# PranjalSahu/tensorflow_distributed

Hardware: AMD Instinct MI355X
Metric: images/sec (whole node) MNIST CNN DP at 1/2/4/8 MI355X; step-time scaling (higher is better)
Workload: dtype bf16; 1 GPU; global_batch=128, per_gpu_batch=128, parallelism=dp1, grad_allreduce=bf16, hipgraph=True, steps_per_graph=20, dp_transport=none, force_dp=False, zero1_fc1=False, fc_grads=bf16

## Files before the change

### csrc/kernels/mnist.hip

```cpp
#include "../common.h"

#include "../gemm.h"
#include "../gemm256.h"
#include "../mnist_layout.h"
#include "../tfd_kernels.h"
#include "../mnist_tail.h"

#include <algorithm>
#include <stdexcept>

constexpr int GEMM_RS = 2;
constexpr int FDX_BK_ = 128;
constexpr int FDW_BK_ = 64;
constexpr int FC1_BK_ = 32;

namespace tfd {
using namespace mnist;

namespace {

__device__ __forceinline__ int data_row(const int* perm, const int64_t* step, int n_data, int B, int b) {
  if (!perm) return b;
  const int64_t s = *step;
  return perm[(int)((s * (int64_t)B + b) % (int64_t)n_data)];
// ... 437 lines not shown
  for (int c = 0; c < NCLS; ++c) part[(q * 64 + r) * NCLS + c] = acc[c];
  __syncthreads();
  for (int i = t; i < OUTG_ROWS * NCLS; i += 256) {
    const int rr = i / NCLS, mm = blk * OUTG_ROWS + rr;
    if (mm <= HID) {
      const size_t o = OFF_OUT + (size_t)mm * NCLS + (i - rr * NCLS);
      const float g =
          part[i] + part[OUTG_ROWS * NCLS + i] + part[2 * OUTG_ROWS * NCLS + i] + part[3 * OUTG_ROWS * NCLS + i];
      if (a.gbf_a) {
        a.gbf_a[o] = f2bf_bits(g);
      } else {
        a.grad[o] = g;
      }
    }
  }
}

struct OnesRowBuf {
  static constexpr bool KC = false;
  const uint16_t* __restrict__ x;
  int k_lim;
  uint32_t nbytes;
  __device__ __forceinline__ uint4 operator()(int mn, int k) const {
    const uint4 v = buf_ld(x, nbytes, (uint32_t)k * FEAT + mn, k < k_lim && mn < FEAT);
    return (mn == FEAT && k < k_lim) ? make_uint4(0x3F80u, 0u, 0u, 0u) : v;
  }
};
static_assert(FEAT % 8 == 0, "the ones row starts a fresh 8-element chunk");

constexpr int FDW_BM = 64, FDW_BN = 64, FDW_BK = FDW_BK_;
constexpr int FDW_PITCH = FDW_BN + 4;
__device__ __forceinline__ void fc1_dw_store(f32x4 (&acc)[2][2], float* cs, float* out, uint16_t* outbf, int m0,
                                             int n0, int M) {
  const int tid = threadIdx.x, lane = tid & 63, w = tid >> 6, wm = w >> 1, wn = w & 1;
#pragma unroll
  for (int i = 0; i < 2; ++i)
#pragma unroll
    for (int j = 0; j < 2; ++j)
#pragma unroll
      for (int r = 0; r < 4; ++r)
        cs[(wm * 32 + 16 * i + 4 * (lane >> 4) + r) * FDW_PITCH + wn * 32 + 16 * j + (lane & 15)] = acc[i][j][r];
  __syncthreads();
#pragma unroll
  for (int q = tid; q < FDW_BM * FDW_BN / 8; q += 256) {
    const int row = q >> 3, ch = q & 7, m = m0 + row;
    if (m >= M) continue;
    const f32x4 lo = *reinterpret_cast<const f32x4*>(cs + row * FDW_PITCH + ch * 8);
    const f32x4 hi = *reinterpret_cast<const f32x4*>(cs + row * FDW_PITCH + ch * 8 + 4);
    const size_t o = (size_t)m * HID + n0 + ch * 8;
    if (outbf) {
      *reinterpret_cast<uint4*>(outbf + o) =
          make_uint4(pack_bf2(lo[0], lo[1]), pack_bf2(lo[2], lo[3]), pack_bf2(hi[0], hi[1]), pack_bf2(hi[2], hi[3]));
    } else {
      *reinterpret_cast<f32x4*>(out + o) = lo;
      *reinterpret_cast<f32x4*>(out + o + 4) = hi;
    }
  }
}
template <class LA, class LB>
__device__ __forceinline__ void fc1_dw_tile(const MnistStepArgs& a, const LA& la, const LB& lb, int m0, int n0, int K,
                                            bf16* smem) {
  f32x4 acc[2][2];
  gemm_mainloop<FDW_BM, FDW_BN, FDW_BK, 2, 2, LA, LB, GEMM_RS>(la, lb, m0, n0, 0, K, smem, acc);
  fc1_dw_store(acc, reinterpret_cast<float*>(smem), a.grad + OFF_WD1, a.gbf_a ? a.gbf_a + OFF_WD1 : nullptr, m0, n0,
               FEAT + 1);
}
__device__ __forceinline__ void fc1_dw_block(const MnistStepArgs& a, int bx, int by, bf16* smem) {
  OnesRowBuf la{a.p2, a.B, (uint32_t)((int64_t)a.B * FEAT * 2)};
  DenseLoaderX<false> lb{a.dh, HID, HID, a.B};
  fc1_dw_tile(a, la, lb, by * FDW_BM, bx * FDW_BN, a.B, smem);
}

constexpr int FDX_BM = 32, FDX_BN = 64, FDX_BK = FDX_BK_, FDX_BN2 = 32;
template <int BN>
__device__ __forceinline__ void fc1_dx_unpool_store(const MnistStepArgs& a, f32x4 (&acc)[FDX_BM / 32][BN / 32],
                                                    float* cs, int m0, int n0) {
  constexpr int PITCH = BN + 4, CPR = BN / 8;
  const int tid = threadIdx.x, lane = tid & 63, w = tid >> 6, wm = w >> 1, wn = w & 1;
  constexpr int WTM = FDX_BM / 2, WTN = BN / 2;
  const int b = tid / CPR, cc = tid % CPR, m = m0 + b;
  const bool live = b < FDX_BM && m < a.B;
  const size_t xo = (size_t)(live ? m : 0) * FEAT + n0 + cc * 8;
  const uint4 pv = *reinterpret_cast<const uint4*>(a.p2 + xo);
  const uint2 iv = *reinterpret_cast<const uint2*>(a.idx2 + xo);
#pragma unroll
  for (int i = 0; i < WTM / 16; ++i)
#pragma unroll
    for (int j = 0; j < WTN / 16; ++j)
#pragma unroll
      for (int r = 0; r < 4; ++r)
        cs[(wm * WTM + 16 * i + 4 * (lane >> 4) + r) * PITCH + wn * WTN + 16 * j + (lane & 15)] = acc[i][j][r];
  __syncthreads();
  if (!live) return;
  const f32x4 lo = *reinterpret_cast<const f32x4*>(cs + b * PITCH + cc * 8);
  const f32x4 hi = *reinterpret_cast<const f32x4*>(cs + b * PITCH + cc * 8 + 4);
  const float v[8] = {lo[0], lo[1], lo[2], lo[3], hi[0], hi[1], hi[2], hi[3]};
  const uint32_t pw[4] = {pv.x, pv.y, pv.z, pv.w};
  uint32_t g[8];
#pragma unroll
  for (int j = 0; j < 8; ++j) {
    const uint32_t p = (pw[j >> 1] >> (16 * (j & 1))) & 0xFFFFu;
    g[j] = p != 0 ? (uint32_t)f2bf_bits(v[j]) : 0u;
  }
  const int pp = n0 >> 6, c0 = (n0 & 63) + cc * 8, ph = pp / 7, pwx = pp - ph * 7;
  const uint32_t iw[2] = {iv.x, iv.y};
#pragma unroll
  for (int wi = 0; wi < 4; ++wi) {
    uint32_t o[4];
#pragma unroll
    for (int q = 0; q < 4; ++q) {
      const uint32_t i0 = (iw[q >> 1] >> (16 * (q & 1))) & 0xFFu, i1 = (iw[q >> 1] >> (16 * (q & 1) + 8)) & 0xFFu;
      o[q] = (i0 == (uint32_t)wi ? g[2 * q] : 0u) | (i1 == (uint32_t)wi ? g[2 * q + 1] << 16 : 0u);
    }
    const int oh = 2 * ph + (wi >> 1), ow = 2 * pwx + (wi & 1);
    *reinterpret_cast<uint4*>(a.dz2 + ((size_t)(m * 14 + oh) * 14 + ow) * 64 + c0) = make_uint4(o[0], o[1], o[2], o[3]);
  }
}
constexpr int FDX_RS = 1, FDX_RS_ALONE = 2;
constexpr int FDXD_BK = 64, FDXD_S = 4;
constexpr int FDXD_A = FDX_BM * FDXD_BK * 2, FDXD_B = FDX_BN * FDXD_BK * 2, FDXD_STAGE = FDXD_A + FDXD_B;
constexpr int FDXD_SMEM = FDXD_S * FDXD_STAGE;
constexpr int FDXD_NK = HID / FDXD_BK;
static_assert(FDX_BM == 32 && FDX_BN == 64 && FDXD_NK >= FDXD_S, "fc1 dX DMA ring geometry");
__device__ __forceinline__ void fdxd_stage(const DenseKC& sa, const DenseKC& sb, char* img, int m0, int n0, int k0,
                                           int w, int l) {
#if defined(__HIP_DEVICE_COMPILE__)
  {
    const int row = w * 8 + (l >> 3);
    __builtin_amdgcn_raw_ptr_buffer_load_lds(sa.rsrc(), (__attribute__((address_space(3))) void*)(img + w * 1024), 16,
                                             sa.off(m0 + row, k0 + kc_slot(row, l & 7) * 8), 0, 0, 0);
  }
#pragma unroll
  for (int i = 0; i < 2; ++i) {
    const int ins = 2 * w + i, row = ins * 8 + (l >> 3);
    __builtin_amdgcn_raw_ptr_buffer_load_lds(sb.rsrc(), (__attribute__((address_space(3))) void*)(img + FDXD_A + ins * 1024),
                                             16, sb.off(n0 + row, k0 + kc_slot(row, l & 7) * 8), 0, 0, 0);
  }
#else
  (void)sa; (void)sb; (void)img; (void)m0; (void)n0; (void)k0; (void)w; (void)l;
#endif
}
__device__ __forceinline__ void fc1_dx_block_dma(const MnistStepArgs& a, int bx, int by, char* smem) {
  const DenseKC sa{a.dh, HID, a.B, HID};
  const DenseKC sb{a.pbf + OFF_WD1, HID, FEAT, HID};
  const int tid = threadIdx.x, l = tid & 63, w = tid >> 6, wm = w >> 1, wn = w & 1;
  const int m0 = by * FDX_BM, n0 = bx * FDX_BN;
  f32x4 acc[1][2] = {{f32x4{0.f, 0.f, 0.f, 0.f}, f32x4{0.f, 0.f, 0.f, 0.f}}};
#pragma unroll
  for (int s = 0; s < FDXD_S - 1; ++s) fdxd_stage(sa, sb, smem + s * FDXD_STAGE, m0, n0, s * FDXD_BK, w, l);
  for (int t = 0; t < FDXD_NK; ++t) {
    const int after = min(FDXD_S - 2, FDXD_NK - 1 - t);
    if (after == 2) asm volatile("s_waitcnt vmcnt(6)" ::: "memory");
    else if (after == 1) asm volatile("s_waitcnt vmcnt(3)" ::: "memory");
    else asm volatile("s_waitcnt vmcnt(0)" ::: "memory");
    __syncthreads();
    if (t + FDXD_S - 1 < FDXD_NK)
      fdxd_stage(sa, sb, smem + ((t + FDXD_S - 1) % FDXD_S) * FDXD_STAGE, m0, n0, (t + FDXD_S - 1) * FDXD_BK, w, l);
    const char* As = smem + (t % FDXD_S) * FDXD_STAGE;
    const char* Bs = As + FDXD_A;
#pragma unroll
    for (int ks = 0; ks < 2; ++ks) {
      const int ch = 4 * ks + (l >> 4);
      const int ra = 16 * wm + (l & 15);
      const bf16x8 af = *reinterpret_cast<const bf16x8*>(As + ra * 128 + (kc_slot(ra, ch) << 4));
#pragma unroll
      for (int j = 0; j < 2; ++j) {
        const int rb = 32 * wn + 16 * j + (l & 15);
        const bf16x8 bf = *reinterpret_cast<const bf16x8*>(Bs + rb * 128 + (kc_slot(rb, ch) << 4));
        acc[0][j] = mfma16x16x32(af, bf, acc[0][j]);
      }
    }
  }
  __syncthreads();
  fc1_dx_unpool_store<FDX_BN>(a, acc, reinterpret_cast<float*>(smem), m0, n0);
}

template <int BN = FDX_BN, int RS = FDX_RS>
__device__ __forceinline__ void fc1_dx_block(const MnistStepArgs& a, int bx, int by, bf16* smem) {
  DenseLoaderX<true> la{a.dh, HID, a.B, HID};
  DenseLoaderX<true> lb{a.pbf + OFF_WD1, HID, FEAT, HID};
  f32x4 acc[FDX_BM / 32][BN / 32];
  gemm_mainloop<FDX_BM, BN, FDX_BK, 2, 2, decltype(la), decltype(lb), RS>(la, lb, by * FDX_BM, bx * BN, 0, HID, smem,
                                                                          acc);
  fc1_dx_unpool_store<BN>(a, acc, reinterpret_cast<float*>(smem), by * FDX_BM, bx * BN);
}

constexpr int FDW_GX = HID / FDW_BN, FDW_GY = (FEAT + 1 + FDW_BM - 1) / FDW_BM;
constexpr int FDX_GX = FEAT / FDX_BN;
constexpr int FDX_GX2 = FEAT / FDX_BN2;
static_assert(FEAT % FDX_BN == 0 && FEAT % FDX_BN2 == 0, "fc1 dX tiles cover the 3136 features exactly");
__device__ __forceinline__ void fdx_tile(int j, int gx, int gy, int& bx, int& by) {
  const int full = (gx * gy) / (8 * gy) * (8 * gy);
  const int T = j < full ? (j & 7) * (full >> 3) + (j >> 3) : j;
  bx = T / gy;
  by = T - bx * gy;
}
__global__ __launch_bounds__(256) void fc1_bwd(MnistStepArgs a, int n_dx, int part) {
  extern __shared__ __attribute__((aligned(16))) char smem_raw[];
  int id = blockIdx.x;
// ... 37 lines not shown
  const int m = blk * OUTS_ROWS + r;
  const int B = a.B, WB = a.sfb_world * B;
  const int per = (WB + OUTS_GROUPS - 1) / OUTS_GROUPS, k0 = min(WB, q * per), k1 = min(WB, k0 + per);
  const int64_t hoff = (int64_t)B * HID, doff = 2 * (int64_t)B * HID;
  float acc[NCLS];
#pragma unroll
  for (int c = 0; c < NCLS; ++c) acc[c] = 0.f;
  if (m <= HID) {
    for (int kb = k0; kb < k1; kb += OUTS_LB) {
      float hv[OUTS_LB];
      const float* dl[OUTS_LB];
#pragma unroll
      for (int u = 0; u < OUTS_LB; ++u) {
        const int k = min(kb + u, k1 - 1), rk = k / B, row = k - rk * B;
        const uint16_t* slot = a.sfb_dr + rk * a.sfb_rs;
        hv[u] = (kb + u < k1) ? (m < HID ? bf2f(slot[hoff + (int64_t)row * HID + m]) : 1.f) : 0.f;
        dl[u] = reinterpret_cast<const float*>(slot + doff) + row * NCLS;
      }
#pragma unroll
      for (int u = 0; u < OUTS_LB; ++u)
#pragma unroll
        for (int c = 0; c < NCLS; ++c) acc[c] = fmaf(hv[u], dl[u][c], acc[c]);
    }
  }
#pragma unroll
  for (int c = 0; c < NCLS; ++c) part[(q * OUTS_ROWS + r) * NCLS + c] = acc[c];
  __syncthreads();
  if (t < OUTS_ROWS * NCLS) {
    const int rr = t / NCLS, c = t - rr * NCLS, mm = blk * OUTS_ROWS + rr;
    float g = 0.f;
#pragma unroll
    for (int qq = 0; qq < OUTS_GROUPS; ++qq) g += part[(qq * OUTS_ROWS + rr) * NCLS + c];
    if (mm <= HID) {
      const size_t o = OFF_OUT + (size_t)mm * NCLS + c;
      if (a.gbf_a) a.gbf_a[o] = f2bf_bits(g);
      else a.grad[o] = g;
    }
  }
}

__device__ __forceinline__ int xcd_grouped_tile(int b, int first, int n) {
  const int x = b & 7;
  const int first_x = first + ((x - first) & 7);
  return x * (n >> 3) + ((b - first_x) >> 3);
}


constexpr int C2D_ROWS = 11, C2D_COLS = 20, C2D_PLANE = 224;
constexpr int C2B_NT = 256;
__device__ __forceinline__ const bf16* c2d_w(const bf16* wt, int rr, int ch) {
  return wt + rr * 64 + ((ch ^ (rr & 7)) << 3);
}
__device__ __forceinline__ uint4 buf_ld_so(const uint16_t* base, uint32_t nbytes, uint32_t voff, uint32_t soff) {
  const __amdgpu_buffer_rsrc_t r = __builtin_amdgcn_make_buffer_rsrc((void*)base, (short)0, (int)nbytes, 0x00020000);
  const i32x4v v = __builtin_amdgcn_raw_buffer_load_b128(r, (int)voff, (int)soff, 0);
  return make_uint4((uint32_t)v[0], (uint32_t)v[1], (uint32_t)v[2], (uint32_t)v[3]);
}
#ifndef C2D_TPS
#define C2D_TPS 5
#endif
constexpr int C2D_NST = 25 / C2D_TPS, C2D_WSTAGE = C2D_TPS * 32 * 64;
static_assert(C2D_NST * C2D_TPS == 25 && C2D_WSTAGE % 512 == 0, "whole W2 stages of 1-KB DMA rows");
constexpr int C2D_SMEM = (8 * C2D_PLANE * 8 + 2 * C2D_WSTAGE) * 2;
static_assert(2 * C2D_SMEM <= 160 * 1024, "two conv2_bwd_lds blocks share a CU (the launch's point)");
static_assert(C2D_PLANE * 16 % 256 == 0 && C2D_PLANE >= C2D_ROWS * C2D_COLS, "dz2 plane");
constexpr int C2D_X_OFF = 8 * C2D_PLANE * 8 * 2;
constexpr int C2D_Z_OFF = C2D_X_OFF;
constexpr int C2D_XS_OFF = C2D_Z_OFF + 448 * 32 * 2;
constexpr int C2D_T_END = C2D_XS_OFF + 5 * 18 * 40 * 2;
static_assert(C2D_T_END <= C2D_SMEM && C2D_XS_OFF % 16 == 0 && (C2D_T_END - C2D_Z_OFF) % 16 == 0, "MFMA tail LDS");
__device__ __forceinline__ int c1w_dz(int px, int c) {
  return px * 32 + (((c >> 3) ^ (2 * ((px >> 3) & 1))) << 3) + (c & 7);
}
#define C2D_STAMP(k)                                                                                     \
  do {                                                                                                   \
    if (TFD_STAMP && a.dbg && threadIdx.x == 0) a.dbg[5 * a.B * 8 + bid * 8 + (k)] = (int64_t)__builtin_amdgcn_s_memtime(); \
  } while (0)
__device__ __forceinline__ void conv2_dgrad_body(const MnistStepArgs& a, const int bid) {
  C2D_STAMP(0);
  extern __shared__ __attribute__((aligned(16))) char smem_raw[];
  bf16* img = (bf16*)smem_raw;
  bf16* wt = img + 8 * C2D_PLANE * 8;
  const int b = bid >> 1, h = bid & 1, t = threadIdx.x;
  const uint16_t* src = a.dz2 + (size_t)b * 196 * 64;
  const uint16_t* wsrc = a.pbf + OFF_WC2;
  const RowPre xr = data_row_pre(a, b);
  auto wdma = [&](int st) {
    constexpr int NI = C2D_WSTAGE / 512;
    static_assert(NI % (C2B_NT / 64) == 0, "whole DMA instructions per wave");
    const int wv = t >> 6, ln = t & 63;
    const uint16_t* s0 = wsrc + st * C2D_WSTAGE;
    bf16* d0 = wt + (st & 1) * C2D_WSTAGE;
#pragma unroll
    for (int k = 0; k < NI / (C2B_NT / 64); ++k) {
      const int ii = wv + (C2B_NT / 64) * k, p = ii * 64 + ln, rr = p >> 3, sl = p & 7;
      __builtin_amdgcn_global_load_lds((const void*)(s0 + rr * 64 + ((sl ^ (rr & 7)) << 3)),
                                       (__attribute__((address_space(3))) void*)(d0 + ii * 64 * 8), 16, 0, 0);
    }
  };
  {
    constexpr int CI = 8 * C2D_PLANE, NI = CI / C2B_NT;
    static_assert(CI % C2B_NT == 0, "whole image chunks per thread");
    wdma(0);
    wdma(1);
    uint4 vi[NI];
#pragma unroll
    for (int j = 0; j < NI; ++j) {
      const int i = t + C2B_NT * j, ch = i / C2D_PLANE, px = i - ch * C2D_PLANE;
      const int r = px / C2D_COLS + 7 * h - 2, c = px % C2D_COLS - 2;
      vi[j] = buf_ld(src, 196 * 64 * 2, (uint32_t)((r * 14 + c) * 64 + ch * 8),
                     px < C2D_ROWS * C2D_COLS && (unsigned)r < 14u && (unsigned)c < 14u);
    }
#pragma unroll
    for (int j = 0; j < NI; ++j) *reinterpret_cast<uint4*>(img + (t + C2B_NT * j) * 8) = vi[j];
  }
  C2D_STAMP(1);
  const int lane = t & 63, w = t >> 6, g = lane >> 4, mt0 = w;
  const int two = (mt0 + 4 < 7);
  float xpre[4];
  uint32_t p1pre[2][2][4];
  uint32_t ipb[2][2][4];
  {
    const float* xrow = a.data + (size_t)data_row_use(a, xr, b) * 784;
#pragma unroll
    for (int q = 0; q < 4; ++q) {
      const int i = 4 * t + q, r = i >> 5, c = i & 31;
      xpre[q] = (r >= 2 && r < 30 && c >= 2 && c < 30) ? xrow[(r - 2) * 28 + c - 2] : 0.f;
    }
  }
#pragma unroll
  for (int j = 0; j < 2; ++j)
#pragma unroll
    for (int nt = 0; nt < 2; ++nt)
#pragma unroll
      for (int r = 0; r < 4; ++r) {
        const int x = min(4 * g + r, 13), n = nt * 16 + (lane & 15), ih = 7 * h + min(mt0 + 4 * j, 6);
        p1pre[j][nt][r] = a.p1[((size_t)b * 196 + ih * 14 + x) * 32 + n];
        ipb[j][nt][r] = a.idx1[((size_t)b * 196 + ih * 14 + x) * 32 + n];
      }
  __syncthreads();
  C2D_STAMP(2);
  const int iw = lane & 15, nl = lane & 15;
  f32x4 acc[2][2];
#pragma unroll
  for (int j = 0; j < 2; ++j) acc[j][0] = acc[j][1] = f32x4{0.f, 0.f, 0.f, 0.f};
  {
    const bf16* a0 = img + ((mt0 + 4) * C2D_COLS + iw + 4) * 8 + g * C2D_PLANE * 8 - (4 * C2D_COLS + 4) * 8;
    const bf16* a1 = a0 + 4 * C2D_COLS * 8;
    const bf16* bw[2][2] = {{c2d_w(wt, nl, g), c2d_w(wt, 16 + nl, g)}, {c2d_w(wt, nl, g + 4), c2d_w(wt, 16 + nl, g + 4)}};
    bf16x8 fb[2][2], fa[2][2];
    auto ld = [&](int st, int slot) {
      const int tap = st >> 1, sk = st & 1;
      const int woff = ((tap / C2D_TPS) & 1) * C2D_WSTAGE + (tap % C2D_TPS) * 32 * 64;
      const int kh = tap / 5, kw = tap - kh * 5, aoff = ((4 - kh) * C2D_COLS + 4 - kw) * 8 + sk * 4 * C2D_PLANE * 8;
      fb[slot][0] = *reinterpret_cast<const bf16x8*>(bw[sk][0] + woff);
      fb[slot][1] = *reinterpret_cast<const bf16x8*>(bw[sk][1] + woff);
      fa[slot][0] = *reinterpret_cast<const bf16x8*>(a0 + aoff);
      fa[slot][1] = *reinterpret_cast<const bf16x8*>(a1 + aoff);
    };
    constexpr int NS = 50, SPS = 2 * C2D_TPS;
    ld(0, 0);
#pragma unroll
    for (int st = 0; st < NS; ++st) {
      const int cur = st & 1;
      if (st + 1 < NS) {
        if ((st + 1) % SPS == 0) {
          __syncthreads();
          if ((st + 1) / SPS + 1 < C2D_NST) wdma((st + 1) / SPS + 1);
        }
        ld(st + 1, cur ^ 1);
      }
#pragma unroll
      for (int j = 0; j < 2; ++j) {
        acc[j][0] = mfma16x16x32(fa[cur][j], fb[cur][0], acc[j][0]);
        acc[j][1] = mfma16x16x32(fa[cur][j], fb[cur][1], acc[j][1]);
      }
    }
  }
#pragma unroll
  for (int j = 0; j < 2; ++j) asm volatile("" : "+v"(acc[j][0]), "+v"(acc[j][1]));
  C2D_STAMP(3);
  __syncthreads();
  for (int i = t; i < (C2D_T_END - C2D_Z_OFF) / 16; i += C2B_NT)
    reinterpret_cast<uint4*>(smem_raw + C2D_Z_OFF)[i] = zero4();
  __syncthreads();
  C2D_STAMP(4);
  {
    bf16* dz1 = reinterpret_cast<bf16*>(smem_raw + C2D_Z_OFF);
    bf16* xsh = reinterpret_cast<bf16*>(smem_raw + C2D_XS_OFF);
#pragma unroll
    for (int j = 0; j < 2; ++j)
#pragma unroll
      for (int nt = 0; nt < 2; ++nt)
#pragma unroll
        for (int r = 0; r < 4; ++r) asm volatile("" : "+v"(p1pre[j][nt][r]), "+v"(ipb[j][nt][r]));
#pragma unroll
    for (int j = 0; j < 2; ++j) {
      if (j == 1 && !two) break;
#pragma unroll
      for (int nt = 0; nt < 2; ++nt) {
        const int n = nt * 16 + (lane & 15), lr = mt0 + 4 * j;
#pragma unroll
        for (int r = 0; r < 4; ++r) {
          const int x = 4 * g + r;
          if (x >= 14) break;
          const int wi = ipb[j][nt][r], px = (2 * lr + (wi >> 1)) * 32 + 2 * x + (wi & 1);
          reinterpret_cast<uint16_t*>(dz1)[c1w_dz(px, n)] = p1pre[j][nt][r] != 0 ? f2bf_bits(acc[j][nt][r]) : (uint16_t)0;
        }
      }
    }
#pragma unroll
    for (int q = 0; q < 4; ++q) {
      const int i = 4 * t + q, r = i >> 5, c = i & 31, rr = r - 14 * h;
      if ((unsigned)rr < 18u) {
        const uint16_t xv = f2bf_bits(xpre[q]);
#pragma unroll
        for (int kw = 0; kw < 5; ++kw)
          if (c >= kw) reinterpret_cast<uint16_t*>(xsh)[(kw * 18 + rr) * 40 + c - kw] = xv;
      }
    }
    __syncthreads();
    C2D_STAMP(5);
    const int mi = w & 1, ni = w >> 1;
    const int tap = 16 * mi + (lane & 15), tc = min(tap, 24), tkh = tc / 5, tkw = tc - 5 * tkh;
    const int q = (lane & 15) >> 2, p4 = lane & 3;
    bf16x8 ones, zer;
#pragma unroll
    for (int e = 0; e < 8; ++e) { ones[e] = (bf16)1.0f; zer[e] = (bf16)0.0f; }
    f32x4 c2 = f32x4{0.f, 0.f, 0.f, 0.f};
#pragma unroll
    for (int ks = 0; ks < 14; ++ks) {
      const int px0 = ks * 32 + 8 * g, rl = px0 >> 5, col0 = px0 & 31;
      bf16x8 af = *reinterpret_cast<const bf16x8*>(xsh + (tkw * 18 + rl + tkh) * 40 + col0);
      if (tap >= 25) af = (tap == 25) ? ones : zer;
      const int row0 = ks * 32 + 8 * g + q, col = 16 * ni + 4 * p4;
      const bf16x8 bfr = frag_tr16(dz1 + c1w_dz(row0, col), dz1 + c1w_dz(row0 + 4, col));
      c2 = mfma16x16x32(af, bfr, c2);
    }
    C2D_STAMP(6);
    const int c = 16 * ni + (lane & 15);
#pragma unroll
    for (int r = 0; r < 4; ++r) {
      const int to = 16 * mi + 4 * g + r;
      if (to < 26) a.wg1_slab[(size_t)bid * 832 + to * 32 + c] = c2[r];
    }
    C2D_STAMP(7);
  }
}

constexpr int C2WL_IMG = 4;
constexpr int C2WL_NTG = 6;
constexpr int C2WL_TPG = 25 / C2WL_NTG;
constexpr int C2WL_MAXT = 25 - C2WL_TPG * (C2WL_NTG - 1);
constexpr int C2WL_CS = 48, C2WL_PW = 18;
constexpr int C2WL_DS = 72, C2WL_KP = 224;
constexpr int C2WL_IMG_ELEMS = C2WL_PW * C2WL_PW * C2WL_CS;
constexpr int C2WL_BRED_OFF = (C2WL_IMG_ELEMS + C2WL_KP * C2WL_DS) * 2;
constexpr int C2WL_SMEM = C2WL_BRED_OFF + 4 * 64 * 4;
static_assert(C2WL_BRED_OFF % 16 == 0 && (C2WL_IMG_ELEMS * 2) % 16 == 0, "LDS carve alignment");
#define C2W_STAMP(k)                                                                                     \
  do {                                                                                                   \
    if (TFD_STAMP && a.dbg && threadIdx.x == 0) a.dbg[7 * a.B * 8 + bid * 8 + (k)] = (int64_t)__builtin_amdgcn_s_memtime(); \
  } while (0)
__device__ __forceinline__ void conv2_wgrad_body(const MnistStepArgs& a, const int bid) {
  C2W_STAMP(0);
  extern __shared__ __attribute__((aligned(16))) char smem_raw[];
  bf16* img = (bf16*)smem_raw;
  bf16* dz = img + C2WL_IMG_ELEMS;
  float* bred = reinterpret_cast<float*>(smem_raw + C2WL_BRED_OFF);
  const int tg = bid % C2WL_NTG, ip = bid / C2WL_NTG, t = threadIdx.x;
  const int tap0 = tg * C2WL_TPG, ntaps = (tg == C2WL_NTG - 1) ? 25 - tap0 : C2WL_TPG;
  const int lane = t & 63, w = t >> 6, h = w >> 1, n0 = 2 * (w & 1), g = lane >> 4, q = (lane & 15) >> 2, p4 = lane & 3;
  constexpr int N1 = (784 + C2B_NT - 1) / C2B_NT, N2 = (1568 + C2B_NT - 1) / C2B_NT;
  uint4 v1[N1], v2[N2];
  auto gload = [&](int b) {
    const uint16_t* s1 = a.p1 + (size_t)b * 196 * 32;
    const uint16_t* s2 = a.dz2 + (size_t)b * 196 * 64;
#pragma unroll
    for (int j = 0; j < N1; ++j) {
      const int i = t + C2B_NT * j;
      v1[j] = (C2B_NT * (j + 1) <= 784) ? buf_ld_so(s1, 196 * 32 * 2, 16u * t, 16u * C2B_NT * j)
                                        : buf_ld(s1, 196 * 32 * 2, 8u * i, i < 784);
    }
#pragma unroll
    for (int j = 0; j < N2; ++j) {
      const int i = t + C2B_NT * j;
      v2[j] = (C2B_NT * (j + 1) <= 1568) ? buf_ld_so(s2, 196 * 64 * 2, 16u * t, 16u * C2B_NT * j)
                                         : buf_ld(s2, 196 * 64 * 2, 8u * i, i < 1568);
    }
  };
  if (ip * C2WL_IMG < a.B) gload(ip * C2WL_IMG);
  for (int i = t; i < C2WL_PW * C2WL_PW; i += C2B_NT) {
    const int r = i / C2WL_PW, c = i - r * C2WL_PW;
    if (r < 2 || r >= 16 || c < 2 || c >= 16) {
      uint4* d = reinterpret_cast<uint4*>(img + i * C2WL_CS);
      d[0] = zero4(); d[1] = zero4(); d[2] = zero4(); d[3] = zero4();
    }
  }
  for (int i = t; i < (C2WL_KP - 196) * (C2WL_DS / 8); i += C2B_NT) reinterpret_cast<uint4*>(dz + 196 * C2WL_DS)[i] = zero4();
  int pos[7][2];
#pragma unroll
  for (int s = 0; s < 7; ++s)
#pragma unroll
    for (int u = 0; u < 2; ++u) {
      const int k = 32 * s + 8 * g + q + 4 * u;
      pos[s][u] = k < 196 ? (k / 14) * C2WL_PW + (k % 14) : 0;
    }
  f32x4 acc[C2WL_MAXT][2];
#pragma unroll
  for (int j = 0; j < C2WL_MAXT; ++j) acc[j][0] = acc[j][1] = f32x4{0.f, 0.f, 0.f, 0.f};
  float bsum = 0.f;
  for (int ii = 0; ii < C2WL_IMG; ++ii) {
    const int b = ip * C2WL_IMG + ii;
    if (b >= a.B) break;
    __syncthreads();
    {
      int tt = t;
      asm volatile("" : "+v"(tt));
#pragma unroll
      for (int j = 0; j < N1; ++j) {
        const int i = tt + C2B_NT * j;
        if (i < 784) {
          const int px = i >> 2, ch = i & 3, r = px / 14, c = px - r * 14;
          *reinterpret_cast<uint4*>(img + ((r + 2) * C2WL_PW + c + 2) * C2WL_CS + ch * 8) = v1[j];
        }
      }
#pragma unroll
      for (int j = 0; j < N2; ++j) {
        const int i = tt + C2B_NT * j;
        if (i < 1568) *reinterpret_cast<uint4*>(dz + (i >> 3) * C2WL_DS + (i & 7) * 8) = v2[j];
      }
    }
    __syncthreads();
    C2W_STAMP(1 + 2 * ii);
    if (ii + 1 < C2WL_IMG && b + 1 < a.B) gload(b + 1);
    if (tg == 0) {
      static_assert(196 % (C2B_NT / 64) == 0, "whole pixel slices");
      const bf16* dzc = dz + (t >> 6) * C2WL_DS + (t & 63);
#pragma unroll 7
      for (int k = 0; k < 196 / (C2B_NT / 64); ++k) bsum += bf2f(dzc[k * (C2B_NT / 64) * C2WL_DS]);
    }
#pragma unroll
    for (int s = 0; s < 7; ++s) {
      bf16x8 bfr[2];
#pragma unroll
      for (int u = 0; u < 2; ++u) {
        const bf16* bp0 = dz + (32 * s + 8 * g + q) * C2WL_DS + 16 * (n0 + u) + 4 * p4;
        bfr[u] = frag_tr16(bp0, bp0 + 4 * C2WL_DS);
      }
#pragma unroll
      for (int j = 0; j < C2WL_MAXT; ++j) {
        if (j < ntaps) {
          const int tap = tap0 + j, toff = (tap / 5) * C2WL_PW + (tap % 5);
          const bf16* a0 = img + (pos[s][0] + toff) * C2WL_CS + 16 * h + 4 * p4;
          const bf16* a1 = img + (pos[s][1] + toff) * C2WL_CS + 16 * h + 4 * p4;
          const bf16x8 af = frag_tr16(a0, a1);
          acc[j][0] = mfma16x16x32(af, bfr[0], acc[j][0]);
          acc[j][1] = mfma16x16x32(af, bfr[1], acc[j][1]);
        }
      }
      __builtin_amdgcn_sched_barrier(0);
    }
    C2W_STAMP(2 + 2 * ii);
  }
#pragma unroll
  for (int j = 0; j < C2WL_MAXT; ++j) asm volatile("" : "+v"(acc[j][0]), "+v"(acc[j][1]));
  float* slab = a.wg2_slab + (size_t)ip * 801 * 64;
#pragma unroll
  for (int j = 0; j < C2WL_MAXT; ++j) {
    if (j < ntaps) {
      const int tap = tap0 + j;
#pragma unroll
      for (int u = 0; u < 2; ++u)
#pragma unroll
        for (int r = 0; r < 4; ++r)
          slab[(size_t)(tap * 32 + 16 * h + 4 * g + r) * 64 + 16 * (n0 + u) + (lane & 15)] = acc[j][u][r];
    }
  }
  if (tg == 0) {
    bred[(t >> 6) * 64 + (t & 63)] = bsum;
    __syncthreads();
    if (t < 64) {
      float sm = 0.f;
#pragma unroll
      for (int sl = 0; sl < C2B_NT / 64; ++sl) sm += bred[sl * 64 + t];
      slab[800 * 64 + t] = sm;
    }
  }
  C2W_STAMP(7);
}

__global__ __launch_bounds__(C2B_NT, 2) void conv2_bwd_lds(MnistStepArgs a, int nw) {
  if ((int)blockIdx.x < nw) {
    conv2_wgrad_body(a, blockIdx.x);
  } else {
    conv2_dgrad_body(a, blockIdx.x - nw);
  }
}

template <int XW>
__device__ __forceinline__ void reduce_chunk(const float* __restrict__ slab, int nslab, int64_t stride, int n, int i0,
                                             float* __restrict__ out, uint16_t* __restrict__ outbf, float* red) {
  constexpr int NY = 256 / XW;
  const int x = threadIdx.x % XW, y = threadIdx.x / XW, i = i0 + x;
  float s = 0.f;
  if (i < n) {
    int k = y;
    for (; k + 3 * NY < nslab; k += 4 * NY) {
      const float v0 = slab[(size_t)k * stride + i], v1 = slab[(size_t)(k + NY) * stride + i];
      const float v2 = slab[(size_t)(k + 2 * NY) * stride + i], v3 = slab[(size_t)(k + 3 * NY) * stride + i];
      s += (v0 + v1) + (v2 + v3);
    }
    for (; k < nslab; k += NY) s += slab[(size_t)k * stride + i];
// ... 159 lines not shown
```

### csrc/runtime/mnist_engine.cpp

```cpp
#include <ATen/ATen.h>
#include <c10/hip/HIPStream.h>
#include <torch/custom_class.h>
#include <torch/library.h>

#include <algorithm>
#include <map>
#include <set>
#include <string>
#include <utility>
#include <vector>

#include "../mnist_layout.h"
#include "../tfd_kernels.h"
#include "comm.h"
#include "ipc_comm.h"

namespace tfd {
using namespace mnist;

#define HIP_OK(x)                                                                          \
  do {                                                                                     \
    hipError_t e_ = (x);                                                                   \
    TORCH_CHECK(e_ == hipSuccess, #x, " failed: ", hipGetErrorString(e_));                 \
  } while (0)

class MnistEngine : public torch::CustomClassHolder {
 public:
  MnistEngine(int64_t batch, int64_t device, double keep_prob, int64_t seed, int64_t rank)
      : B_(batch), device_(device), keep_prob_(keep_prob), seed_((uint32_t)seed), rank_((uint32_t)rank) {
    TORCH_CHECK(batch > 0 && batch <= 65536, "bad batch");
    auto f32 = at::TensorOptions().dtype(at::kFloat).device(at::kCUDA, device);
    auto bf = at::TensorOptions().dtype(at::kBFloat16).device(at::kCUDA, device);
    auto u8 = at::TensorOptions().dtype(at::kByte).device(at::kCUDA, device);
    auto i64 = at::TensorOptions().dtype(at::kLong).device(at::kCUDA, device);
    auto i32 = at::TensorOptions().dtype(at::kInt).device(at::kCUDA, device);
    params_ = at::zeros({TOTAL}, f32);
    pbf_ = at::zeros({TOTAL}, bf);
    grad_ = at::zeros({TOTAL}, f32);
    m_ = at::zeros({TOTAL}, f32);
    v_ = at::zeros({TOTAL}, f32);
    gbf_ = at::zeros({TOTAL}, bf);
    step_ = at::zeros({1}, i64);
    tnext_ = at::zeros({1}, i64);
    fc1_splits_ = mnist_fc1_splits((int)B_);
    wg2_splits_ = mnist_wg2_splits((int)B_);
    p1_ = at::empty({B_, P1H, P1H, C1}, bf);
    idx1_ = at::empty({B_, P1H, P1H, C1}, u8);
    p2_ = at::empty({B_, FEAT}, bf);
    idx2_ = at::empty({B_, FEAT}, u8);
    fc1_slab_ = at::empty({fc1_splits_, B_, HID}, f32);
    hd_ = at::empty({B_, HID}, bf);
    dh_ = at::empty({B_, HID}, bf);
    dlogits_ = at::empty({B_, NCLS}, f32);
    loss_row_ = at::zeros({B_}, f32);
    correct_row_ = at::zeros({B_}, f32);
    dz2_ = at::empty({B_, P1H, P1H, C2}, bf);
    wg2_slab_ = at::empty({wg2_splits_, 801, C2}, f32);
    wg1_slab_ = at::empty({2 * B_, 832}, f32);
    xbuf_ = at::zeros({B_, 784}, f32);
    rows_ = at::full({B_ + 1}, -1, i32);
    xpre_ = at::zeros({B_, 784}, f32);
    ypre_ = at::zeros({B_}, i32);
    ybuf_ = at::zeros({B_}, i32);
    HIP_OK(hipSetDevice((int)device));
    HIP_OK(hipStreamCreateWithFlags(&comm_stream_, hipStreamNonBlocking));
    HIP_OK(hipEventCreateWithFlags(&ev_a_, hipEventDisableTiming));
    HIP_OK(hipEventCreateWithFlags(&ev_b_, hipEventDisableTiming));
    HIP_OK(hipEventCreateWithFlags(&ev_done_, hipEventDisableTiming));
    HIP_OK(hipStreamCreateWithFlags(&opt_stream_, hipStreamNonBlocking));
    HIP_OK(hipEventCreateWithFlags(&ev_opt_a_, hipEventDisableTiming));
    HIP_OK(hipEventCreateWithFlags(&ev_start_, hipEventDisableTiming));
    HIP_OK(hipEventCreateWithFlags(&ev_ag_, hipEventDisableTiming));
    HIP_OK(hipEventCreateWithFlags(&ev_p2_, hipEventDisableTiming));
    HIP_OK(hipEventCreateWithFlags(&ev_wag_, hipEventDisableTiming));
    for (auto& e : pev_) HIP_OK(hipEventCreate(&e));
  }
  ~MnistEngine() override {
    for (auto& kv : graphs_) hipGraphExecDestroy(kv.second);
    hipEventDestroy(ev_a_);
    hipEventDestroy(ev_b_);
    hipEventDestroy(ev_done_);
    hipStreamDestroy(comm_stream_);
    hipStreamDestroy(opt_stream_);
    hipEventDestroy(ev_opt_a_);
    hipEventDestroy(ev_start_);
    hipEventDestroy(ev_ag_);
    hipEventDestroy(ev_p2_);
    hipEventDestroy(ev_wag_);
    for (auto& e : pev_) hipEventDestroy(e);
  }

  at::Tensor params() { return params_; }
  at::Tensor params_bf16() { return pbf_; }
  at::Tensor grads() { return grad_; }
  at::Tensor grads_bf16() { return gbf_; }
  at::Tensor adam_m() { return m_; }
  at::Tensor adam_v() { return v_; }
  at::Tensor step_tensor() { return step_; }
  at::Tensor loss_rows() { return loss_row_; }
  at::Tensor correct_rows() { return correct_row_; }
  at::Tensor hidden() {
    if (fp32_) return fhd_;
    if (sfb_active()) return sfdr_.narrow(0, rank_in_comm() * sfb_rs_ + B_ * HID, B_ * HID).view({B_, HID});
    return hd_;
  }
  at::Tensor pool2() {
    if (sfb_active()) return sfp2_.narrow(0, rank_in_comm() * B_ * FEAT, B_ * FEAT).view({B_, FEAT});
    return p2_;
  }
  at::Tensor pool1() { return p1_; }
  at::Tensor feed_x() { return xbuf_; }
  at::Tensor feed_y() { return ybuf_; }
  int64_t batch() { return B_; }

  void set_dataset(at::Tensor data, at::Tensor labels, at::Tensor perm) {
    TORCH_CHECK(data.is_cuda() && data.scalar_type() == at::kFloat && data.dim() == 2 && data.size(1) == 784,
                "dataset must be a [N,784] fp32 GPU tensor");
    TORCH_CHECK(labels.is_cuda() && labels.scalar_type() == at::kInt && labels.numel() == data.size(0),
                "labels must be [N] int32 GPU");
    TORCH_CHECK(perm.is_cuda() && perm.scalar_type() == at::kInt && perm.numel() == data.size(0),
                "perm must be [N] int32 GPU");
    data_ = data.contiguous();
    labels_ = labels.contiguous();
    perm_ = perm.contiguous();
    invalidate_prefetch();
  }
  void invalidate_prefetch() { rows_.narrow(0, B_, 1).fill_(-1); }
  void set_debug_buffer(at::Tensor t) { dbg_ = t; }
  void set_input_mode(int64_t mode) {
    TORCH_CHECK(mode == 0 || (mode == 1 && data_.defined()), "set_dataset first");
    input_mode_ = mode;
  }
  void set_keep_prob(double kp) { keep_prob_ = kp; }
  void sync_shadow() {
    cast_f32_bf16((const float*)params_.data_ptr(), (uint16_t*)pbf_.data_ptr(), TOTAL, stream());
  }

  void set_adam(double lr, double b1, double b2, double eps) {
    opt_ = 0; b1_ = b1; b2_ = b2; eps_ = eps;
// ... 768 lines not shown
  bool fused_bf16_a() const { return bf16_comm_ && dp(); }
  bool in_gbf(int64_t beg) const { return fused_bf16_a() && beg >= BUCKET_SPLIT; }

  void reduce_bucket(int64_t beg, int64_t end, bool pre) {
    const size_t n = (size_t)(end - beg);
    if (ipc_ && (!comm_ || (int64_t)n <= ipc_small_)) {
      void* out = bf16_comm_ ? (void*)((uint16_t*)gbf_.data_ptr() + beg) : (void*)((float*)grad_.data_ptr() + beg);
      const void* in = pre ? (const void*)((const uint16_t*)gbf_.data_ptr() + beg)
                           : (const void*)((const float*)grad_.data_ptr() + beg);
      ipc_->all_reduce_raw(in, pre, out, bf16_comm_, (int64_t)n, 1.0, comm_stream_);
      return;
    }
    TORCH_CHECK(comm_, "no communicator for a ", n, "-element bucket");
    if (bf16_comm_) {
      uint16_t* gb = (uint16_t*)gbf_.data_ptr() + beg;
      if (!pre) cast_f32_bf16((const float*)grad_.data_ptr() + beg, gb, (int64_t)n, comm_stream_);
      comm_->all_reduce_raw(gb, n, ncclBfloat16, ncclSum, comm_stream_);
    } else {
      comm_->all_reduce_raw((float*)grad_.data_ptr() + beg, n, ncclFloat32, ncclSum, comm_stream_);
    }
  }

  MnistF32Args args_f32() {
    TORCH_CHECK(f1_.defined(), "set_dtype('fp32') first");
    MnistStepArgs a = args();
    MnistF32Args f{};
    f.B = a.B;
    f.data = a.data;
    f.labels = a.labels;
    f.perm = a.perm;
    f.n_data = a.n_data;
    f.step = a.step;
    f.p32 = a.p32;
    f.grad = a.grad;
    f.p1 = (float*)f1_.data_ptr();
    f.idx1 = a.idx1;
    f.p2 = (float*)f2_.data_ptr();
    f.idx2 = a.idx2;
    f.fc1_slab = (float*)fslab_.data_ptr();
    f.hd = (float*)fhd_.data_ptr();
    f.dh = (float*)fdh_.data_ptr();
    f.dlogits = a.dlogits;
    f.loss_row = a.loss_row;
    f.correct_row = a.correct_row;
    f.dz2 = (float*)fdz2_.data_ptr();
    f.wg2_slab = (float*)fwg2_.data_ptr();
    f.wg1_slab = a.wg1_slab;
    f.fc1_splits = mnist_f32_fc1_splits();
    f.wg2_splits = mnist_f32_wg2_splits((int)B_);
    f.keep_prob = a.keep_prob;
    f.seed = a.seed;
    f.rank = a.rank;
    return f;
  }

  MnistStepArgs args() {
    MnistStepArgs a{};
    a.B = (int)B_;
    if (input_mode_ == 1) {
      a.data = (const float*)data_.data_ptr();
      a.labels = (const int*)labels_.data_ptr();
      a.perm = (const int*)perm_.data_ptr();
      a.n_data = (int)data_.size(0);
    } else {
      a.data = (const float*)xbuf_.data_ptr();
      a.labels = (const int*)ybuf_.data_ptr();
      a.perm = nullptr;
      a.n_data = (int)B_;
    }
    a.step = (const int64_t*)step_.data_ptr();
    a.p32 = (const float*)params_.data_ptr();
    a.pbf = (const uint16_t*)pbf_.data_ptr();
    a.grad = (float*)grad_.data_ptr();
    a.p1 = (uint16_t*)p1_.data_ptr();
    a.idx1 = (uint8_t*)idx1_.data_ptr();
    a.p2 = (uint16_t*)p2_.data_ptr();
    a.idx2 = (uint8_t*)idx2_.data_ptr();
    a.fc1_slab = (float*)fc1_slab_.data_ptr();
    a.hd = (uint16_t*)hd_.data_ptr();
    a.dh = (uint16_t*)dh_.data_ptr();
    a.dlogits = (float*)dlogits_.data_ptr();
    a.loss_row = (float*)loss_row_.data_ptr();
    a.correct_row = (float*)correct_row_.data_ptr();
    a.dz2 = (uint16_t*)dz2_.data_ptr();
    a.wg2_slab = (float*)wg2_slab_.data_ptr();
    a.wg1_slab = (float*)wg1_slab_.data_ptr();
    a.fc1_splits = fc1_splits_;
    a.wg2_splits = wg2_splits_;
    a.keep_prob = (float)keep_prob_;
    a.seed = seed_;
    a.rank = rank_;
    a.rows = input_mode_ == 1 ? (int*)rows_.data_ptr() : nullptr;
    a.xpre = input_mode_ == 1 ? (float*)xpre_.data_ptr() : nullptr;
    a.ypre = input_mode_ == 1 ? (int*)ypre_.data_ptr() : nullptr;
    a.dbg = dbg_.defined() ? (int64_t*)dbg_.data_ptr() : nullptr;
    if (sfb_active()) {
      const int64_t r = rank_in_comm();
      uint16_t* slot = (uint16_t*)sfdr_.data_ptr() + r * sfb_rs_;
      a.p2 = (uint16_t*)sfp2_.data_ptr() + r * B_ * FEAT;
      a.dh = slot;
      a.hd = slot + B_ * HID;
      a.dlogits = reinterpret_cast<float*>(slot + 2 * B_ * HID);
      a.sfb_world = (int)world();
      a.sfb_p2 = (const uint16_t*)sfp2_.data_ptr();
      a.sfb_dr = (const uint16_t*)sfdr_.data_ptr();
      a.sfb_rs = sfb_rs_;
    }
    a.sfb_by_lo = 0;
    a.sfb_by_hi = -1;
    return a;
  }

  int64_t B_, device_;
  double keep_prob_;
  uint32_t seed_, rank_;
  int fc1_splits_, wg2_splits_;
  int64_t input_mode_ = 0;
  int opt_ = 0;
  double b1_ = 0.9, b2_ = 0.999, eps_ = 1e-8, momentum_ = 0.0;
  LrSchedule sched_ = lr_constant(0.01f);
  bool nesterov_ = false;
  bool bf16_comm_ = true;
  c10::intrusive_ptr<RcclComm> comm_;
  c10::intrusive_ptr<IpcComm> ipc_;
  int64_t ipc_small_ = 0;
  bool ipc_gather_ = true;
  at::Tensor params_, pbf_, grad_, m_, v_, gbf_, step_, tnext_;
  at::Tensor p1_, idx1_, p2_, idx2_, fc1_slab_, hd_, dh_, dlogits_, loss_row_, correct_row_, dz2_, wg2_slab_,
      wg1_slab_, xbuf_, ybuf_;
  at::Tensor data_, labels_, perm_, rows_, xpre_, ypre_, dbg_;
  at::Tensor f1_, f2_, fhd_, fdh_, fdz2_, fslab_, fwg2_;
  bool fp32_ = false;
  hipStream_t comm_stream_ = nullptr;
  hipEvent_t ev_a_ = nullptr, ev_b_ = nullptr, ev_done_ = nullptr;
  hipStream_t opt_stream_ = nullptr;
  hipEvent_t ev_opt_a_ = nullptr, ev_start_ = nullptr, ev_ag_ = nullptr;
  bool zero_ = false;
  bool merge_tail_ = false;
  bool pending_wag_ = false;
  bool wag_issued_ = false;
  bool force_dp_ = false;
  int64_t zshard_ = 0;
  bool pending_opt_a_ = false;
  bool sfb_ = false;
  at::Tensor sfp2_, sfdr_;
  int64_t sfb_rs_ = 0;
  hipEvent_t ev_p2_ = nullptr, ev_wag_ = nullptr;
  bool fuse_tail_ = true;
  bool local_bf16_grads_ = false;
  std::map<std::string, hipGraphExec_t> graphs_;
  bool topo_ = false;
  int64_t topo_step_ = 0;
  std::set<hipGraphNode_t> topo_seen_;
  std::vector<std::pair<std::string, std::vector<hipGraphNode_t>>> topo_tags_;
  std::string drop_wait_;
  hipEvent_t pev_[P_N] = {};
  bool timing_ = false, timed_ = false, timed_dp_ = false;
};

TORCH_LIBRARY_FRAGMENT(tfd, m) {
  m.class_<RcclComm>("RcclComm")
      .def(torch::init<at::Tensor, int64_t, int64_t, int64_t>())
      .def_static("unique_id", &RcclComm::unique_id)
      .def_static("reap", &RcclComm::reap)
      .def_static("retired_count", &RcclComm::retired_count)
      .def("graph_refs", &RcclComm::graph_refs)
      .def("world", &RcclComm::world)
      .def("rank", &RcclComm::rank)
      .def("all_reduce", &RcclComm::all_reduce)
      .def("reduce_scatter", &RcclComm::reduce_scatter)
      .def("all_gather", &RcclComm::all_gather)
      .def("broadcast", &RcclComm::broadcast)
      .def("send", &RcclComm::send)
      .def("recv", &RcclComm::recv)
      .def("abort", &RcclComm::abort);
  m.class_<MnistEngine>("MnistEngine")
      .def(torch::init<int64_t, int64_t, double, int64_t, int64_t>())
      .def("params", &MnistEngine::params)
      .def("params_bf16", &MnistEngine::params_bf16)
      .def("grads", &MnistEngine::grads)
      .def("grads_bf16", &MnistEngine::grads_bf16)
      .def("adam_m", &MnistEngine::adam_m)
      .def("adam_v", &MnistEngine::adam_v)
      .def("step_tensor", &MnistEngine::step_tensor)
      .def("loss_rows", &MnistEngine::loss_rows)
      .def("correct_rows", &MnistEngine::correct_rows)
      .def("hidden", &MnistEngine::hidden)
      .def("pool1", &MnistEngine::pool1)
      .def("pool2", &MnistEngine::pool2)
      .def("feed_x", &MnistEngine::feed_x)
      .def("feed_y", &MnistEngine::feed_y)
      .def("batch", &MnistEngine::batch)
      .def("set_dataset", &MnistEngine::set_dataset)
      .def("invalidate_prefetch", &MnistEngine::invalidate_prefetch)
      .def("set_debug_buffer", &MnistEngine::set_debug_buffer)
      .def("set_input_mode", &MnistEngine::set_input_mode)
      .def("set_keep_prob", &MnistEngine::set_keep_prob)
      .def("sync_shadow", &MnistEngine::sync_shadow)
      .def("set_adam", &MnistEngine::set_adam)
      .def("set_momentum", &MnistEngine::set_momentum)
      .def("set_lr_schedule", &MnistEngine::set_lr_schedule)
      .def("lr_at_step", &MnistEngine::lr_at_step)
      .def("set_comm", &MnistEngine::set_comm)
      .def("set_ipc", &MnistEngine::set_ipc)
      .def("set_ipc_gather", &MnistEngine::set_ipc_gather)
      .def("set_zero", &MnistEngine::set_zero)
      .def("set_sfb_merge_reduce", &MnistEngine::set_sfb_merge_reduce)
      .def("sfb_merge_reduce", &MnistEngine::sfb_merge_reduce)
      .def("set_fc_sfb", &MnistEngine::set_fc_sfb)
      .def("fc_sfb", &MnistEngine::fc_sfb)
      .def("sfb_shard_elems", &MnistEngine::sfb_shard_elems)
// ... 30 lines not shown
```

### csrc/tfd_kernels.h

```cpp
#pragma once
#include <hip/hip_runtime_api.h>
#include <stdint.h>

#include "lr_schedule.h"

namespace tfd {

struct MnistStepArgs {
  int B;
  const float* data;
  const int* labels;
  const int* perm;
  int n_data;
  const int64_t* step;
  int64_t* t_out;
  int64_t* step_bump;
  const float* p32;
  const uint16_t* pbf;
  float* grad;
  uint16_t* gbf_a;
  uint16_t* gbf_b;
  uint16_t* p1;  uint8_t* idx1;
  uint16_t* p2;  uint8_t* idx2;
  float* fc1_slab;
  uint16_t* hd;  uint16_t* dh;
  float* dlogits;
  float* loss_row; float* correct_row;
  uint16_t* dz2;
  float* wg2_slab;
  float* wg1_slab;
  int fc1_splits, wg2_splits;
  float keep_prob;
  uint32_t seed, rank;
  int* rows;
  float* xpre;
  int* ypre;
  int64_t* dbg;
  int sfb_world;
  const uint16_t* sfb_p2;
  const uint16_t* sfb_dr;
  int64_t sfb_rs;
  int sfb_by_lo, sfb_by_hi;
};

int mnist_fc1_splits(int B);
int mnist_wg2_splits(int B);
void mnist_forward(const MnistStepArgs& a, bool train, hipStream_t s);
void mnist_forward_conv(const MnistStepArgs& a, hipStream_t s);
void mnist_forward_fc(const MnistStepArgs& a, bool train, hipStream_t s);
void mnist_backward_a(const MnistStepArgs& a, hipStream_t s, int part = 0);
void mnist_backward_b(const MnistStepArgs& a, hipStream_t s);
void mnist_conv_grad_reduce(const MnistStepArgs& a, hipStream_t s);

struct MnistAdamArgs {
  float* p; float* m; float* v;
  uint16_t* pbf;
  LrSchedule sched;
  float beta1, beta2, eps;
  const int64_t* t;
  int64_t* step;
  const uint16_t* gbf;
};
void mnist_adam_fused(const MnistStepArgs& a, const MnistAdamArgs& o, hipStream_t s, bool fc_region = true);
void mnist_fc_grad_sfb(const MnistStepArgs& a, hipStream_t s, bool with_reduce = false);
void mnist_sfb_tile_rows(int row0, int row1, int* by_lo, int* by_hi);
int64_t mnist_sfb_slot_elems(int B);

struct MnistF32Args {
  int B;
  const float* data; const int* labels; const int* perm; int n_data;
  const int64_t* step;
  const float* p32;
  float* grad;
  float* p1; uint8_t* idx1;
  float* p2; uint8_t* idx2;
  float* fc1_slab;
  float* hd; float* dh;
  float* dlogits;
  float* loss_row; float* correct_row;
  float* dz2;
  float* wg2_slab;
  float* wg1_slab;
  int fc1_splits, wg2_splits;
  float keep_prob;
  uint32_t seed, rank;
  int64_t* t_out;
};
int mnist_f32_fc1_splits();
int mnist_f32_wg2_splits(int B);
void mnist_f32_forward(const MnistF32Args& a, bool train, hipStream_t s);
void mnist_f32_backward(const MnistF32Args& a, hipStream_t s);

struct AdamArgs {
  float* p; float* m; float* v; const float* g; uint16_t* pbf;
  const uint16_t* gbf;
  int64_t n;
  LrSchedule sched;
  float beta1, beta2, eps;
  const int64_t* step;
  int t_offset;
  float grad_scale;
};
void adam_apply(const AdamArgs& a, hipStream_t s);
void adam_apply_ranges(const AdamArgs& a, int nr, const int64_t* beg, const int64_t* n, hipStream_t s);
struct SgdArgs {
  float* p; float* mom; const float* g; uint16_t* pbf; const uint16_t* gbf; int64_t n;
  LrSchedule sched;
  float momentum, weight_decay, grad_scale; int nesterov;
  const int64_t* step;
  int t_offset;
};
// ... 13 lines not shown
```

Baseline: 2.182 million images/s.

## Store pooled-resolution conv2 gradient and unpool on the fly in consumers

The fc1 dX epilogue now writes the masked gradient at pooled resolution (dp2, B×FEAT) instead of scattering a 4x-larger unpooled dz2 tensor. The conv2 dgrad and conv2 wgrad kernels instead load dp2 together with the 8-bit argmax indices and expand them into LDS using a shift-based select. This cuts global write and read traffic for the pooling backward by roughly 4x. In exchange the consumers do extra index loads and ALU work, and the dgrad kernel now zero-fills padding separately from the unpool writes.

```diff
diff --git a/csrc/kernels/mnist.hip b/csrc/kernels/mnist.hip
--- a/csrc/kernels/mnist.hip
+++ b/csrc/kernels/mnist.hip
@@ -543,7 +543,6 @@
   const bool live = b < FDX_BM && m < a.B;
   const size_t xo = (size_t)(live ? m : 0) * FEAT + n0 + cc * 8;
   const uint4 pv = *reinterpret_cast<const uint4*>(a.p2 + xo);
-  const uint2 iv = *reinterpret_cast<const uint2*>(a.idx2 + xo);
 #pragma unroll
   for (int i = 0; i < WTM / 16; ++i)
 #pragma unroll
@@ -563,19 +562,37 @@
     const uint32_t p = (pw[j >> 1] >> (16 * (j & 1))) & 0xFFFFu;
     g[j] = p != 0 ? (uint32_t)f2bf_bits(v[j]) : 0u;
   }
-  const int pp = n0 >> 6, c0 = (n0 & 63) + cc * 8, ph = pp / 7, pwx = pp - ph * 7;
-  const uint32_t iw[2] = {iv.x, iv.y};
-#pragma unroll
-  for (int wi = 0; wi < 4; ++wi) {
-    uint32_t o[4];
-#pragma unroll
-    for (int q = 0; q < 4; ++q) {
-      const uint32_t i0 = (iw[q >> 1] >> (16 * (q & 1))) & 0xFFu, i1 = (iw[q >> 1] >> (16 * (q & 1) + 8)) & 0xFFu;
-      o[q] = (i0 == (uint32_t)wi ? g[2 * q] : 0u) | (i1 == (uint32_t)wi ? g[2 * q + 1] << 16 : 0u);
-    }
-    const int oh = 2 * ph + (wi >> 1), ow = 2 * pwx + (wi & 1);
-    *reinterpret_cast<uint4*>(a.dz2 + ((size_t)(m * 14 + oh) * 14 + ow) * 64 + c0) = make_uint4(o[0], o[1], o[2], o[3]);
-  }
+  *reinterpret_cast<uint4*>(a.dp2 + xo) =
+      make_uint4(g[0] | g[1] << 16, g[2] | g[3] << 16, g[4] | g[5] << 16, g[6] | g[7] << 16);
+}
+typedef short s16x2 __attribute__((ext_vector_type(2)));
+struct UnpoolSel {
+  s16x2 s[4];
+};
+__device__ __forceinline__ UnpoolSel unpool_sel(const uint2& iv) {
+  UnpoolSel r;
+#pragma unroll
+  for (int q = 0; q < 4; ++q) {
+    const uint32_t lanes = __builtin_amdgcn_perm(0u, q < 2 ? iv.x : iv.y, (q & 1) ? 0x0C030C02u : 0x0C010C00u);
+    r.s[q] = s16x2{(short)0x1000, (short)0x1000} << __builtin_bit_cast(s16x2, lanes);
+  }
+  return r;
+}
+__device__ __forceinline__ uint4 unpool_chunk(const uint4& gv, const UnpoolSel& sel, int wi) {
+  const uint32_t gw[4] = {gv.x, gv.y, gv.z, gv.w};
+  uint32_t o[4];
+#pragma unroll
+  for (int q = 0; q < 4; ++q) {
+    const s16x2 sh = {(short)(3 - wi), (short)(3 - wi)}, s15 = {15, 15};
+    o[q] = gw[q] & __builtin_bit_cast(uint32_t, (sel.s[q] << sh) >> s15);
+  }
+  return make_uint4(o[0], o[1], o[2], o[3]);
+}
+typedef int i32x2v __attribute__((ext_vector_type(2)));
+__device__ __forceinline__ uint2 buf_ld8(const uint8_t* base, uint32_t nbytes, uint32_t off, bool ok) {
+  const __amdgpu_buffer_rsrc_t r = __builtin_amdgcn_make_buffer_rsrc((void*)base, (short)0, (int)nbytes, 0x00020000);
+  const i32x2v v = __builtin_amdgcn_raw_buffer_load_b64(r, ok ? off : kBufOOB, 0, 0);
+  return make_uint2((uint32_t)v[0], (uint32_t)v[1]);
 }
 constexpr int FDX_RS = 1, FDX_RS_ALONE = 2;
 constexpr int FDXD_BK = 64, FDXD_S = 4;
@@ -779,7 +796,8 @@
   bf16* img = (bf16*)smem_raw;
   bf16* wt = img + 8 * C2D_PLANE * 8;
   const int b = bid >> 1, h = bid & 1, t = threadIdx.x;
-  const uint16_t* src = a.dz2 + (size_t)b * 196 * 64;
+  const uint16_t* gsrc = a.dp2 + (size_t)b * FEAT;
+  const uint8_t* isrc = a.idx2 + (size_t)b * FEAT;
   const uint16_t* wsrc = a.pbf + OFF_WC2;
   const RowPre xr = data_row_pre(a, b);
   auto wdma = [&](int st) {
@@ -796,20 +814,41 @@
     }
   };
   {
-    constexpr int CI = 8 * C2D_PLANE, NI = CI / C2B_NT;
+    constexpr int CI = 8 * C2D_PLANE, NI = CI / C2B_NT, NE = 5 * 7 * 8, NP = (NE + C2B_NT - 1) / C2B_NT;
     static_assert(CI % C2B_NT == 0, "whole image chunks per thread");
     wdma(0);
     wdma(1);
-    uint4 vi[NI];
+    uint4 gv[NP];
+    uint2 iv[NP];
+    int prow[NP], pcol[NP], cch[NP];
+#pragma unroll
+    for (int j = 0; j < NP; ++j) {
+      const int e = t + C2B_NT * j;
+      pcol[j] = e % 7;
+      cch[j] = (e / 7) & 7;
+      prow[j] = e / 56;
+      const uint32_t o = (uint32_t)(((2 * h + prow[j]) * 7 + pcol[j]) * 64 + cch[j] * 8);
+      gv[j] = buf_ld(gsrc, FEAT * 2, o, e < NE);
+      iv[j] = buf_ld8(isrc, FEAT, o, e < NE);
+    }
 #pragma unroll
     for (int j = 0; j < NI; ++j) {
-      const int i = t + C2B_NT * j, ch = i / C2D_PLANE, px = i - ch * C2D_PLANE;
+      const int i = t + C2B_NT * j, px = i % C2D_PLANE;
       const int r = px / C2D_COLS + 7 * h - 2, c = px % C2D_COLS - 2;
-      vi[j] = buf_ld(src, 196 * 64 * 2, (uint32_t)((r * 14 + c) * 64 + ch * 8),
-                     px < C2D_ROWS * C2D_COLS && (unsigned)r < 14u && (unsigned)c < 14u);
-    }
-#pragma unroll
-    for (int j = 0; j < NI; ++j) *reinterpret_cast<uint4*>(img + (t + C2B_NT * j) * 8) = vi[j];
+      if (!(px < C2D_ROWS * C2D_COLS && (unsigned)r < 14u && (unsigned)c < 14u))
+        *reinterpret_cast<uint4*>(img + i * 8) = zero4();
+    }
+#pragma unroll
+    for (int j = 0; j < NP; ++j) {
+      if (t + C2B_NT * j >= NE) continue;
+      const UnpoolSel sel = unpool_sel(iv[j]);
+#pragma unroll
+      for (int wi = 0; wi < 4; ++wi) {
+        const int ir = 2 * (2 * h + prow[j]) + (wi >> 1) - (7 * h - 2), ic = 2 * pcol[j] + (wi & 1) + 2;
+        if ((unsigned)ir < (unsigned)C2D_ROWS)
+          *reinterpret_cast<uint4*>(img + (cch[j] * C2D_PLANE + ir * C2D_COLS + ic) * 8) = unpool_chunk(gv[j], sel, wi);
+      }
+    }
   }
   C2D_STAMP(1);
   const int lane = t & 63, w = t >> 6, g = lane >> 4, mt0 = w;
@@ -968,11 +1007,13 @@
   const int tg = bid % C2WL_NTG, ip = bid / C2WL_NTG, t = threadIdx.x;
   const int tap0 = tg * C2WL_TPG, ntaps = (tg == C2WL_NTG - 1) ? 25 - tap0 : C2WL_TPG;
   const int lane = t & 63, w = t >> 6, h = w >> 1, n0 = 2 * (w & 1), g = lane >> 4, q = (lane & 15) >> 2, p4 = lane & 3;
-  constexpr int N1 = (784 + C2B_NT - 1) / C2B_NT, N2 = (1568 + C2B_NT - 1) / C2B_NT;
+  constexpr int N1 = (784 + C2B_NT - 1) / C2B_NT, N2 = (392 + C2B_NT - 1) / C2B_NT;
   uint4 v1[N1], v2[N2];
+  uint2 vx[N2];
   auto gload = [&](int b) {
     const uint16_t* s1 = a.p1 + (size_t)b * 196 * 32;
-    const uint16_t* s2 = a.dz2 + (size_t)b * 196 * 64;
+    const uint16_t* s2 = a.dp2 + (size_t)b * FEAT;
+    const uint8_t* sx = a.idx2 + (size_t)b * FEAT;
 #pragma unroll
     for (int j = 0; j < N1; ++j) {
       const int i = t + C2B_NT * j;
@@ -982,8 +1023,9 @@
 #pragma unroll
     for (int j = 0; j < N2; ++j) {
       const int i = t + C2B_NT * j;
-      v2[j] = (C2B_NT * (j + 1) <= 1568) ? buf_ld_so(s2, 196 * 64 * 2, 16u * t, 16u * C2B_NT * j)
-                                         : buf_ld(s2, 196 * 64 * 2, 8u * i, i < 1568);
+      v2[j] = (C2B_NT * (j + 1) <= 392) ? buf_ld_so(s2, FEAT * 2, 16u * t, 16u * C2B_NT * j)
+                                        : buf_ld(s2, FEAT * 2, 8u * i, i < 392);
+      vx[j] = buf_ld8(sx, FEAT, 8u * i, i < 392);
     }
   };
   if (ip * C2WL_IMG < a.B) gload(ip * C2WL_IMG);
@@ -1025,7 +1067,14 @@
 #pragma unroll
       for (int j = 0; j < N2; ++j) {
         const int i = tt + C2B_NT * j;
-        if (i < 1568) *reinterpret_cast<uint4*>(dz + (i >> 3) * C2WL_DS + (i & 7) * 8) = v2[j];
+        if (i < 392) {
+          const int pp = i >> 3, ph = pp / 7, pw = pp - ph * 7;
+          bf16* d = dz + ((2 * ph) * 14 + 2 * pw) * C2WL_DS + (i & 7) * 8;
+          const UnpoolSel sel = unpool_sel(vx[j]);
+#pragma unroll
+          for (int wi = 0; wi < 4; ++wi)
+            *reinterpret_cast<uint4*>(d + ((wi >> 1) * 14 + (wi & 1)) * C2WL_DS) = unpool_chunk(v2[j], sel, wi);
+        }
       }
     }
     __syncthreads();
diff --git a/csrc/runtime/mnist_engine.cpp b/csrc/runtime/mnist_engine.cpp
--- a/csrc/runtime/mnist_engine.cpp
+++ b/csrc/runtime/mnist_engine.cpp
@@ -54,7 +54,7 @@
     dlogits_ = at::empty({B_, NCLS}, f32);
     loss_row_ = at::zeros({B_}, f32);
     correct_row_ = at::zeros({B_}, f32);
-    dz2_ = at::empty({B_, P1H, P1H, C2}, bf);
+    dp2_ = at::empty({B_, FEAT}, bf);
     wg2_slab_ = at::empty({wg2_splits_, 801, C2}, f32);
     wg1_slab_ = at::empty({2 * B_, 832}, f32);
     xbuf_ = at::zeros({B_, 784}, f32);
@@ -989,7 +989,7 @@
     a.dlogits = (float*)dlogits_.data_ptr();
     a.loss_row = (float*)loss_row_.data_ptr();
     a.correct_row = (float*)correct_row_.data_ptr();
-    a.dz2 = (uint16_t*)dz2_.data_ptr();
+    a.dp2 = (uint16_t*)dp2_.data_ptr();
     a.wg2_slab = (float*)wg2_slab_.data_ptr();
     a.wg1_slab = (float*)wg1_slab_.data_ptr();
     a.fc1_splits = fc1_splits_;
@@ -1033,7 +1033,7 @@
   int64_t ipc_small_ = 0;
   bool ipc_gather_ = true;
   at::Tensor params_, pbf_, grad_, m_, v_, gbf_, step_, tnext_;
-  at::Tensor p1_, idx1_, p2_, idx2_, fc1_slab_, hd_, dh_, dlogits_, loss_row_, correct_row_, dz2_, wg2_slab_,
+  at::Tensor p1_, idx1_, p2_, idx2_, fc1_slab_, hd_, dh_, dlogits_, loss_row_, correct_row_, dp2_, wg2_slab_,
       wg1_slab_, xbuf_, ybuf_;
   at::Tensor data_, labels_, perm_, rows_, xpre_, ypre_, dbg_;
   at::Tensor f1_, f2_, fhd_, fdh_, fdz2_, fslab_, fwg2_;
diff --git a/csrc/tfd_kernels.h b/csrc/tfd_kernels.h
--- a/csrc/tfd_kernels.h
+++ b/csrc/tfd_kernels.h
@@ -26,7 +26,7 @@
   uint16_t* hd;  uint16_t* dh;
   float* dlogits;
   float* loss_row; float* correct_row;
-  uint16_t* dz2;
+  uint16_t* dp2;
   float* wg2_slab;
   float* wg1_slab;
   int fc1_splits, wg2_splits;
```

New measurement: 2.194 million images/s, median of 6. No clear change (+0.5%).
